# EMI-Group/evogp

Hardware: AMD Instinct MI355X
Metric: tree_evals_per_s (higher is better)
Workload: dtype f32; 1 GPU; BASELINE north_star / configs[2] shape: SymbolicRegression synthetic 10-var, GLOBAL pop=1000000 x 1024 datapoints, max_tree_len=64, funcs + - * /, one tree_SR_fitness pass over every rank's shard per step; global_pop=1000000, pop_per_gpu=1000000, datapoints=1024, var_len=10, max_tree_len=64, ranks=1, device_prewarm_calls=40

## Files before the change

evogp_amd/_lib.py:

```python
from __future__ import annotations

import ctypes as C
import os

_HERE = os.path.dirname(os.path.abspath(__file__))
LIB_PATH = os.environ.get("EVOGP_HIP_LIB") or os.path.join(_HERE, "lib", "libevogp_hip.so")

ABI_VERSION = 9

_vp = C.c_void_p
_u = C.c_uint
_i = C.c_int
_f = C.c_float

PROTOTYPES = {
    "evogp_hip_generate": [_u, _u, _u, _u, _u, _f, _f, _vp, _vp, _vp, _vp, _vp, _vp, _vp, _u, _vp],
    "evogp_hip_mutate": [_i, _i, _vp, _vp, _vp, _vp, _vp, _vp, _vp, _vp, _vp, _vp, _vp],
    "evogp_hip_crossover": [_i, _i, _i, _vp, _vp, _vp, _vp, _vp, _vp, _vp, _vp, _vp, _vp, _vp],
    "evogp_hip_evaluate": [_u, _u, _u, _u, _vp, _vp, _vp, _vp, _vp, _vp],
    "evogp_hip_sr_fitness": [_u, _u, _u, _u, _u, _i, _vp, _vp, _vp, _vp, _vp, _vp, _u, _vp],
    "evogp_hip_generate_masked": [_u, _u, _u, _u, _u, _f, _f, _vp, _vp, _vp, _vp, _vp, _vp, _vp, _u, _vp, _u, _vp],
    "evogp_hip_breed_default": [_i, _i, _i, _i, _vp, _vp, _vp, _vp, _vp, _u, _vp, _vp, _vp, _vp, _vp, _vp, _vp, _vp],
    "evogp_hip_breed_default_rows": [_i, _i, _i, _i, _vp, _vp, _vp, _vp, _vp, _u, _vp, _vp, _vp, _vp, _vp, _vp, _vp, _i, _i, _vp],
    "evogp_hip_breed_default_table": [_i, _i, _i, _i, _i, _vp, _vp, _vp, _vp, _vp, _u, _vp, _vp, _vp, _vp, _vp, _vp, _vp, _i, _i, _vp],
# ... 11 lines not shown
    "evogp_hip_random_words": [C.c_longlong, C.c_longlong, _i, C.c_longlong, C.c_longlong, C.c_longlong, _vp, _vp],
    "evogp_hip_fitness_scores": [_u, _i, _vp, _vp, _vp],
    "evogp_hip_select": [_u, _u, _u, _vp, _vp, _vp, _vp],
    "evogp_hip_select_alternating": [_u, _u, _u, _vp, _vp, _vp, _vp, _vp],
    "evogp_hip_tournament_select": [_u, _u, _u, C.c_longlong, C.c_longlong, _vp, _vp, _vp],
    "evogp_hip_set_program_buffer_limit": [C.c_ulonglong],
    "evogp_hip_release_workspaces": [],
    "evogp_hip_set_allocator": [_vp, _vp],
    "evogp_hip_set_sr_division": [C.c_int],
    "evogp_hip_get_sr_division": [],
    "evogp_hip_abi_version": [],
    "evogp_hip_sr_gradient": [_u, _u, _u, _u, _u, _i, _vp, _vp, _vp, _vp, _vp, _vp, _vp, _vp],
    "evogp_hip_sr_const_step": [_u, _u, _u, _i, _vp, _vp, _vp, _vp, _vp, _vp, _vp, _vp, _vp, _vp],
    "evogp_hip_sr_case_errors": [_u, _u, _u, _u, _u, _i, _vp, _vp, _vp, _vp, _vp, _vp, _vp],
    "evogp_hip_lexicase_workspace_bytes": [_u, _u, _u, C.POINTER(C.c_ulonglong)],
    "evogp_hip_lexicase_select": [_u, _u, _vp, _vp, _u, C.c_longlong, C.c_longlong, _vp, _vp, _vp],
    "evogp_hip_pareto_rank_workspace_bytes": [_u, C.POINTER(C.c_ulonglong)],
    "evogp_hip_pareto_rank": [_u, _u, _vp, _vp, _vp, _vp, _vp, _vp, _vp],
    "evogp_hip_nsga2_select": [_u, _vp, _u, _u, _u, C.c_longlong, C.c_longlong, _vp, _vp],
    "evogp_hip_sr_subtree_errors": [_u, _u, _u, _u, _u, _i, _vp, _vp, _vp, _vp, _vp, _vp, _vp, _vp],
    "evogp_hip_prune_rows": [_u, _u, _u, _i, _i, _vp, _vp, _vp, _vp, _vp, _vp, _vp, _vp, _vp, _vp, _vp],
    "evogp_hip_sr_normal_eq": [_u, _u, _u, _u, _u, _vp, _vp, _vp, _vp, _vp, _vp, _vp, _vp],
    "evogp_hip_sr_lm_step": [_u, _u, _u, _i, _vp, _vp, _vp, _vp, _vp, _vp, _vp, _vp, _vp, _vp],
}

DEBUG_PROTOTYPES = {
    "evogp_hip_timer_begin": [_vp],
    "evogp_hip_timer_end": [_vp, C.POINTER(C.c_float)],
    "evogp_hip_debug_set_stats": [_vp],
    "evogp_hip_debug_compile_batch": [_i],
    "evogp_hip_debug_long_compiler": [_i],
    "evogp_hip_debug_twins": [_i],
    "evogp_hip_debug_tc_fold": [_i],
    "evogp_hip_debug_profile": [_i],
    "evogp_hip_debug_profile_read": [C.POINTER(C.c_float), C.POINTER(C.c_int)],
    "evogp_hip_debug_tc_histogram": [_u, _vp, _i, _vp],
    "evogp_hip_debug_tc_nhandlers": [],
    "evogp_hip_debug_tc_program": [_u, _vp, _i],
    "evogp_hip_debug_forget_function_classes": [],
    "evogp_hip_debug_structural_mutate_given": [_i, _i, _i, _i, _i, _vp, _vp, _vp, _vp, _vp, _vp, _vp, _vp],
    "evogp_hip_debug_insert_mutate_given": [_i, _i, _i, _vp, _vp, _vp, _vp, _vp, _vp, _vp, _vp, _vp, _vp, _vp],
    "evogp_hip_debug_point_mutate_given": [_i, _i, _i, _i, _i, _i, _i, _i, _i, _vp, _vp, _vp, _vp, _vp, _vp, _vp, _vp, _vp, _vp, _vp, _vp, _vp, _vp],
    "evogp_hip_debug_lexicase": [_vp, _i],
    "evogp_hip_debug_pareto_rank": [_i],
}


def _load() -> C.CDLL:
    if not os.path.exists(LIB_PATH):
        raise ImportError(
            f"{LIB_PATH} is missing: build the HIP engine first "
            "(python -c 'import __graft_entry__ as g; g.build()'  or  make -C evogp_amd/csrc). "
            "evogp_amd has no CPU fallback."
        )
    lib = C.CDLL(LIB_PATH)
    for name, argtypes in list(PROTOTYPES.items()) + list(DEBUG_PROTOTYPES.items()):
        fn = getattr(lib, name)
        fn.argtypes = argtypes
        fn.restype = _i
    lib.evogp_hip_evaluate_workspace_bytes.argtypes = [_u, _u]
    lib.evogp_hip_evaluate_workspace_bytes.restype = C.c_size_t
    lib.evogp_hip_select_workspace_bytes.argtypes = []
    lib.evogp_hip_select_workspace_bytes.restype = C.c_size_t
    lib.evogp_hip_program_buffer_bytes.argtypes = []
    lib.evogp_hip_program_buffer_bytes.restype = C.c_ulonglong
    lib.evogp_hip_record_ring_bytes.argtypes = []
# ... 16 lines not shown
```

evogp_amd/csrc/sr_tc.hip:

```cpp
#include "interp.hpp"
#include "launch.hpp"
#include "sr_params.hpp"
#include "tc_interp_k8.inc"
#include "tc_interp_k4.inc"
#include "tc_interp_k1.inc"

#include <atomic>
#include <cstddef>
#include <mutex>
#include <cstdio>
#include <vector>

namespace evogp {

struct TcCompileParams {
    const float *value;
    const int16_t *type;
    const int16_t *size;
    uint2 *prog;
    float *fitness;
    unsigned *marks;
    unsigned *zero_next;
    int pop, gp_len, var_len;
    uint32_t unary_mask;
// ... 2 lines not shown
    uint32_t rec;
    uint32_t overflow;
    int depth;
    int out_len;
    int nblocks;
    int rows;
    int general;
    int heavy_reserve;
    int div_reserve;
    int classify;
    uint32_t recip;
    int twins;
    int long_fast;
    int learn;
    int nan_trees;
};

__device__ inline uint32_t division_in_place(uint32_t id, int after, const TcCompileParams &p) {
    if (id < 24u || id >= 32u) return id;
    const uint32_t form = id - 24u;
    const uint32_t ip = form == 0u ? (uint32_t)EVOGP_TC_H_DIVIP_SS : form == 3u ? (uint32_t)EVOGP_TC_H_DIVIP_SC : form == 4u ? (uint32_t)EVOGP_TC_H_DIVIP_CS : 0u;
    if (ip == 0u) return id;
    const int before = after + (form == 0u ? 1 : 0);
    return before + p.div_reserve <= p.depth ? ip : id;
}

enum : int { TC_S = 0, TC_V = 1, TC_C = 2 };
constexpr int kMarkSampleBlocks = 64;
constexpr int kZeroRounds = 3;
static std::atomic<int> g_long_fast{-1};
static std::atomic<int> g_twins{-1};
static std::atomic<int> g_fold{-1};
static std::atomic<int> g_compile_batch{-2};
static int tc_nan_trees() {
    static const int env_fold = env_int("EVOGP_TC_FOLD", 2);
    const int fo = g_fold.load(std::memory_order_relaxed);
    return fo >= 0 ? fo : (env_fold < 0 || env_fold > 2 ? 2 : env_fold);
}
static_assert(kSentinelHeavy == 0x7FC0FEEDu, "gen/gen_tc_asm.py SENTINEL_HEAVY");

__device__ inline float fold_bin4_fast(int op, float x, float y) {
    return op == 0 ? x + y : op == 1 ? x - y : op == 2 ? x * y : (y == 0.0f ? __builtin_nanf("") : x / y);
}

__device__ inline uint32_t tc_word0(int id, int slot, uint32_t pf_bytes, uint32_t aux = 0u) {
    return ((pf_bytes >> 10) << 24) | ((aux & 0xFFu) << 16) | (uint32_t)(((slot & 1) * EVOGP_TC_NHANDLERS + id) * EVOGP_TC_SLOT);
}

static_assert(EVOGP_TC_H_PUSH_V == EVOGP_TC_H_PUSH_C + 1 && EVOGP_TC_H_DIVIP_CS == EVOGP_TC_H_DIVIP_SS + 2 && EVOGP_TC_H_DIVR_CV == EVOGP_TC_H_DIVR_SV + 2 &&
              EVOGP_TC_H_PUSH_C_NP == EVOGP_TC_H_ADD_SS_NP + 24 && EVOGP_TC_H_DIVIP_SS_NP == EVOGP_TC_H_ADD_SS_NP + 26 &&
              EVOGP_TC_H_DIVR_SV_NP == EVOGP_TC_H_ADD_SS_NP + 29, "gen/gen_tc_asm.py NOPF_TWINS");
__device__ inline int no_prefetch_delta(bool arith3, bool push_c, bool in_place, bool by_recip) {
    return arith3 ? (int)EVOGP_TC_H_ADD_SS_NP : push_c ? (int)EVOGP_TC_H_PUSH_C_NP - (int)EVOGP_TC_H_PUSH_C
         : in_place ? (int)EVOGP_TC_H_DIVIP_SS_NP - (int)EVOGP_TC_H_DIVIP_SS : by_recip ? (int)EVOGP_TC_H_DIVR_SV_NP - (int)EVOGP_TC_H_DIVR_SV : 0;
}
__device__ inline bool next_word_has_variable(const TcCompileParams &, unsigned long long keptwave, bool kept, bool uses_var, bool is_root) {
    const unsigned long long U = __ballot(kept & uses_var);
    return __builtin_amdgcn_inverse_ballot_w64((((~keptwave) + (U << 1)) & keptwave) | __ballot(is_root));
}

__device__ inline void division_by_reciprocal(const TcCompileParams &p, int &id, uint32_t pf, uint32_t d1, uint32_t &aux) {
    const bool sv = id == 3 * 8 + 1, vv = id == 3 * 8 + 5, cv = id == 3 * 8 + 7;
    const bool ok = (p.recip != 0u) & (sv | vv | cv);
    const uint32_t voff = vv ? d1 << 4 : pf;
    aux = ok ? (voff + p.recip) >> 10 : aux;
    id = ok ? (int)EVOGP_TC_H_DIVR_SV + (int)vv + 2 * (int)cv : id;
// ... 378 lines not shown
        Mpz &= B((MU & segmask) == 0ull);
    }
    const M Mhigh = B(hf > p.depth);
    M Mlong = 0ull;
    if (U0) Mlong = Mroot & B(slot + 1 > 31);
    int cls = TREE_OK;
    if ((Min & (~(Mleaf | M4) | Msb | Mhigh | Mlong)) != 0ull) {
        const M segmask = L(Min) ? ((len >= 64 ? ~0ull : ((1ull << len) - 1ull)) << lo) : 0ull;
        auto seg_any = [&](M m) -> bool { return (m & segmask) != 0ull; };
        cls = seg_any(Min & B(kind == 3)) ? TREE_HEAVY : seg_any(Min & B(kind == 5)) ? TREE_GENERAL : seg_any(Min & Msb) ? TREE_HEAVY
            : seg_any(Min & Mhigh) ? (p.gp_len > 64 && p.general ? TREE_GENERAL : TREE_HEAVY) : seg_any(Mlong) ? TREE_HEAVY : TREE_OK;
    }
    const M Mdivown = MB & ~Mpushc & ~Mdivr & B(opx == 3);
    const M Mss = Mdivown & B(form == 0), Msc = Mdivown & B(form == 3), Mcs = Mdivown & B(form == 4);
    const int ip = seli(L(Mss), (int)EVOGP_TC_H_DIVIP_SS, seli(L(Msc), (int)EVOGP_TC_H_DIVIP_SC, (int)EVOGP_TC_H_DIVIP_CS));
    const M Minpl = (Mss | Msc | Mcs) & B(hf + seli(L(Mss), 1, 0) + p.div_reserve <= p.depth);
    id = seli(L(Minpl), ip, id);
    if (p.twins) {
        const M Muses = ~Mpushc & ~MU & ((MB & (MlV | MrV)) | (~MB & MV));
        const M Uk = Mkept & Muses;
        const M nxt = (((~keptwave) + (Uk << 1)) & keptwave) | Mroot;
        id += seli(L(nxt), 0, no_prefetch_delta(L(MB & ~Mpushc & ~Mdivr & B(opx < 3)), L(Mpushc), L(Minpl), L(Mdivr & ~Mpushc)));
    }
    const M Mok = B(cls == TREE_OK);
    if (L(Mkept & Mok & ~Mpz)) *(uint2 *)(rec0 + (roff + (uint32_t)slot * 8u)) = make_uint2(tc_word0(id, slot, pf, aux), d1);
    if (L(Mroot)) {
        uint32_t skip = tc_word0(EVOGP_TC_H_SKIP, 0, 0u), nan_tree = tc_word0(EVOGP_TC_H_NAN_TREE, 0, 0u);
        asm volatile("" : "+v"(skip), "+v"(nan_tree));
        const uint32_t last = selu(L(Mpz), nan_tree, tc_word0(EVOGP_TC_H_END, slot + 1, p.ydelta));
        *(uint2 *)(rec0 + (roff + (uint32_t)seli(L(Mok & ~Mpz), slot + 1, 0) * 8u)) = make_uint2(selu(L(Mok), last, skip), 0u);
    }
    if (cls == TREE_GENERAL && !p.general) cls = TREE_HEAVY;
    return L(Min) ? cls : (int)TREE_OK;
}

template <bool U0>
__device__ inline int compile_pack_arith_plain(const TcCompileParams &p, char *rec0, uint32_t roff, bool in, int lo, int len, int ty, int sz, float val, int lane) {
    auto bperm = [](int v, int i4) -> int { return __builtin_amdgcn_ds_bpermute(i4, v); };
    auto next = [](int v) -> int { return __builtin_amdgcn_update_dpp(0, v, 0x130 , 0xf, 0xf, true); };
    auto any = [](bool c) -> bool { return __builtin_amdgcn_ballot_w64(c) != 0ull; };
    auto seli = [](bool c, int x, int y) -> int { return c ? x : y; };
    auto selu = [](bool c, uint32_t x, uint32_t y) -> uint32_t { return c ? x : y; };
    auto self = [](bool c, float x, float y) -> float { return c ? x : y; };
    const int end = lo + len;
    const uint32_t f = (uint32_t)val;
    const bool isV = ty == T_VAR, isC = ty == T_CONST, isBf = ty == T_BFUNC;
    const uint32_t opu = f - (uint32_t)F_ADD;
    const bool is4 = isBf & (opu < 4u);
    const bool g5 = (isBf & (f - (uint32_t)F_LOOSE_DIV <= (uint32_t)(F_GE - F_LOOSE_DIV))) | (ty == T_TFUNC) | (ty == T_UFUNC);
    const int v = max(0, min((int)val, p.var_len - 1));
    const uint32_t pay = selu(isV, (uint32_t)v * p.var_stride, f2bits(val));
    const bool u0 = U0 && in & (ty == T_UFUNC) & (f - (uint32_t)F_SIN > (uint32_t)(F_LOOSE_SQRT - F_SIN)) & (p.unary_mask != 0u);
    const int kind = seli(isV, 0, seli(isC, 1, seli(is4, 2, seli(u0, 4, seli(g5, 5, 3)))));
    const int op = (int)(opu & 3u);
    const bool isB = in & (kind == 2), isU = U0 && u0;
    const int ks = kind | (sz << 3);
    const int ksl = next(ks);
    const int szl = ksl >> 3;
    const int ri = lane + 1 + szl, ri4 = ri << 2;
    const int ksr = bperm(ks, ri4);
    const int szr = ksr >> 3;
    const bool size_bad = (sz != seli(isB, 1 + szl + szr, seli(isU, 1 + szl, 1))) | (isB & ((szl < 1) | (ri >= end))) | (isU & ((szl < 1) | (lane + 1 >= end)));
    int kl = ksl & 7, kr = ksr & 7;
    uint32_t pl = (uint32_t)next((int)pay), pr = (uint32_t)bperm((int)pay, ri4);
    auto fold = [&](uint32_t a, uint32_t b, bool who) -> uint32_t {
        const float x = bits2f(a), y = bits2f(b);
// ... 1054 lines not shown
                if (ty == T_VAR) {
                    int v = (int)val;
                    v = v < 0 ? 0 : (v >= p.var_len ? p.var_len - 1 : v);
                    pf = (uint32_t)v * p.var_stride; d1 = 0u;
                }
                rec[0] = make_uint2(tc_word0(ty == T_VAR ? EVOGP_TC_H_PUSH_V : EVOGP_TC_H_PUSH_C, 0, pf), d1);
                rec[1] = make_uint2(tc_word0(EVOGP_TC_H_END, 1, p.ydelta), 0u);
            }
            continue;
        }
        if (len <= 0) cls = TREE_BAD;
        else if (len <= 64) {
            if (__any(lane < len && ty == T_UFUNC && p.unary_mask != 0u)) cls = compile_tree<true>(p, rec, len, ty, sz, val, lane);
            else cls = compile_tree_arith(p, rec, len, ty, sz, val, lane);
        }
        if (cls == TREE_GENERAL && !p.general) cls = TREE_HEAVY;
        if (cls != TREE_OK && lane == 0) {
            rec[0] = make_uint2(tc_word0(EVOGP_TC_H_SKIP, 0, 0u), 0u);
            p.fitness[t] = cls == TREE_BAD ? __builtin_nanf("") : bits2f(cls == TREE_GENERAL ? kSentinelGeneral : kSentinelHeavy);
            if (cls == TREE_GENERAL && p.marks) p.marks[4] = 1u;
            else if (cls == TREE_HEAVY && p.marks) {
                p.marks[0] = 1u;
                if (blockIdx.x < kMarkSampleBlocks) atomicAdd(p.marks + 2, 1u);
            }
        }
    }
}

__device__ inline bool generic_node(int ty, float val) {
    const uint32_t f = (uint32_t)val;
    return (ty == T_TFUNC) | ((ty == T_BFUNC) & (f - (uint32_t)F_ADD >= 4u)) | ((ty == T_UFUNC) & ((f == (uint32_t)F_LOOSE_INV) | (f - (uint32_t)F_SINH <= 2u)));
}

template <int B, int MODE, bool LONGROWS>
__global__ __launch_bounds__(256) void tc_compile_packed_kernel(TcCompileParams p) {
    constexpr bool UN = MODE != 0;
    const int lane = threadIdx.x & 63;
    if (p.zero_next && blockIdx.x == 0)
        for (int i = threadIdx.x; i < kCallScratchWords; i += blockDim.x) p.zero_next[i] = 0u;
    const uint32_t wave_id = uni((blockIdx.x * blockDim.x + threadIdx.x) >> 6);
    const uint32_t t0 = wave_id * (uint32_t)B;
    if (t0 >= (uint32_t)p.pop) return;
    const int nb = (int)min((uint32_t)B, (uint32_t)p.pop - t0);
    const int L = p.gp_len;
    int raw = 1;
    if (lane < nb) raw = (int)p.size[(size_t)(t0 + (uint32_t)lane) * L];
    char *const rec0 = (char *)p.prog + (size_t)t0 * p.rec;
    const bool longer = LONGROWS && lane < nb && min(raw, L) > 64;
    if (LONGROWS && longer) {
        uint32_t skip = tc_word0(EVOGP_TC_H_SKIP, 0, 0u);
        asm volatile("" : "+v"(skip));
        *(uint2 *)(rec0 + (uint32_t)__mul24(lane, (int)p.rec)) = make_uint2(skip, 0u);
        p.fitness[t0 + (uint32_t)lane] = bits2f(p.general ? kSentinelGeneral : kSentinelHeavy);
        if (p.marks) {
            if (p.general) {
                const int n = min(raw, L);
                p.marks[p.long_fast ? 8 + (int)(n > 128) + (int)(n > 256) + (int)(n > 512) : 4] = 1u;
            }
            else {
                p.marks[0] = 1u;
                if ((wave_id >> 2) < (uint32_t)kMarkSampleBlocks) atomicAdd(p.marks + 2, 1u);
            }
        }
    }
    const int lens = lane < nb && !longer ? max(1, min(raw, L)) : 0;
    int sval = lens | (raw <= 0 ? 128 : 0) | (lane << 8);
#pragma unroll
    for (int r = 3; r < 7; ++r) {
        const unsigned long long ones = __builtin_amdgcn_ballot_w64((sval & (1 << r)) != 0);
        const int below1 = (int)__builtin_amdgcn_mbcnt_hi((uint32_t)(ones >> 32), __builtin_amdgcn_mbcnt_lo((uint32_t)ones, 0u));
        const int to = (sval & (1 << r)) ? below1 : __popcll(ones) + lane - below1;
        sval = __builtin_amdgcn_ds_permute(to << 2, sval);
    }
    const int slen = sval & 127;
    const size_t node0 = (size_t)t0 * (uint32_t)L;
    const float *const value0 = p.value + node0;
    const int16_t *const type0 = p.type + node0, *const size0 = p.size + node0;
    unsigned long long left = LONGROWS ? __builtin_amdgcn_ballot_w64(slen > 0) : (nb >= 64 ? ~0ull : (1ull << nb) - 1ull);
    bool n_in = false;
    unsigned long long n_inm = 0ull;
    int n_tb = 0, n_lo = 0, n_len = 0, n_bad = 0, n_ty = T_CONST, n_sz = 1;
    float n_val = 0.0f;
    auto plan = [&]() {
        int used = 0, about = 0;
        while (true) {
            const unsigned long long cand = __builtin_amdgcn_ballot_w64(slen <= 64 - used) & left;
            if (cand == 0ull) break;
            const int j = __builtin_ctzll(cand);
            left &= ~(1ull << j);
            const int sv = __builtin_amdgcn_readlane(sval, j), l = sv & 127;
            about = (uint32_t)(lane - used) < (uint32_t)l ? (sv | (used << 16)) : about;
            used += l;
            if (used >= 64) break;
        }
        n_in = lane < used;
        n_inm = used >= 64 ? ~0ull : (1ull << used) - 1ull;
        n_tb = (about >> 8) & 255; n_lo = about >> 16; n_len = about & 127; n_bad = about & 128;
        n_ty = T_CONST; n_sz = 1; n_val = 0.0f;
        if (n_in) {
            const uint32_t at = (uint32_t)(__mul24(n_tb, L) + lane - n_lo);
            n_ty = (int)*(const int16_t *)((const char *)type0 + at * 2u); n_val = *(const float *)((const char *)value0 + at * 4u);
            n_sz = (int)*(const int16_t *)((const char *)size0 + at * 2u);
        }
    };
    bool more = left != 0ull;
    if (more) plan();
    uint32_t seen = 0u;
    while (more) {
        const bool in = n_in;
        const unsigned long long inm = n_inm;
        const int tb = n_tb, lo = n_lo, len = n_len, bad = n_bad, sz = n_sz;
        const int ty = bad ? -1 : n_ty;
        const float val = n_val;
        more = left != 0ull;
        if (more) plan();
        const uint32_t roff = (uint32_t)__mul24(tb, (int)p.rec);
        int cls;
        const bool unary = __builtin_amdgcn_ballot_w64(ty == T_UFUNC) != 0ull;
        if (MODE == 3) cls = compile_pack_mo(p, rec0, roff, in, lo, len, ty, sz, val, lane);
        else if (MODE == 2 && __builtin_amdgcn_ballot_w64(generic_node(ty, val)) != 0ull) cls = compile_pack_generic(p, rec0, roff, in, lo, len, ty, sz, val, lane);
        else if (UN && unary && p.unary_mask != 0u) cls = compile_pack_unary<true>(p, rec0, roff, in, lo, len, ty, sz, val, lane);
        else if (!UN && unary) cls = compile_pack_arith<true>(p, rec0, roff, inm, lo, len, ty, sz, val, lane);
        else cls = compile_pack_arith<false>(p, rec0, roff, inm, lo, len, ty, sz, val, lane);
        if (MODE != 3 && p.learn) {
            const bool look = MODE != 0 || __builtin_amdgcn_ballot_w64(cls != TREE_OK) != 0ull;
            if (look) {
                const bool gen = __builtin_amdgcn_ballot_w64(generic_node(ty, val)) != 0ull;
                const bool un = unary && __builtin_amdgcn_ballot_w64((ty == T_UFUNC) & ((uint32_t)val - (uint32_t)F_SIN <= (uint32_t)(F_LOOSE_SQRT - F_SIN))) != 0ull;
                seen |= ((un | gen) ? 1u : 0u) | (gen ? 2u : 0u);
            }
        }
        if (cls != TREE_OK && in && lane == lo) {
            const bool nan = bad != 0 || cls == TREE_BAD;
            p.fitness[t0 + (uint32_t)tb] = nan ? __builtin_nanf("") : bits2f(cls == TREE_GENERAL ? kSentinelGeneral : kSentinelHeavy);
            if (!nan && p.marks) {
                if (cls == TREE_GENERAL) p.marks[p.long_fast ? 8 : 4] = 1u;
                else {
                    p.marks[0] = 1u;
                    if ((wave_id >> 2) < (uint32_t)kMarkSampleBlocks) atomicAdd(p.marks + 2, 1u);
                }
            }
        }
    }
    if (MODE != 3 && p.learn && p.marks && uni((int)seen) != 0 && lane == 0) {
        p.marks[5] = 1u;
        if (seen & 2u) p.marks[6] = 1u;
    }
}
// ... 980 lines not shown
            long sample = 0;
            for (long w = 0; w < sw && w < n; ++w) sample += (n - 1 - w) / nwaves + 1;
            *mark_sample = (int)sample;
        }
        const size_t clds = 4 * tc_general_lds_bytes(p.gp_len);
        if (clds > 64 * 1024 && !d.attr_set[15]) {
            (void)hipFuncSetAttribute((const void *)tc_compile_general_kernel<true>, hipFuncAttributeMaxDynamicSharedMemorySize, 160 * 1024 - 1024);
            (void)hipGetLastError();
            d.attr_set[15] = true;
        }
        static const int env_packed_env = env_int("EVOGP_TC_PACKED", -1);
        const int set_packed = g_compile_batch.load(std::memory_order_relaxed);
        const int env_packed = set_packed != -2 ? set_packed : env_packed_env;
        static const int env_generic = env_int("EVOGP_TC_PACK_GENERIC", 1);
        const bool packed_mo = p.out_len > 1 && env_packed != 0 && env_generic != 0;
        const bool packed = (p.out_len == 1 && env_packed != 0) || packed_mo;
        if (packed) {
            const bool un = c.nblocks != 1;
            constexpr unsigned kOwnHandlers = (1u << F_ADD) | (1u << F_SUB) | (1u << F_MUL) | (1u << F_DIV) | (1u << F_SIN) | (1u << F_COS) | (1u << F_TAN) |
                                              (1u << F_LOG) | (1u << F_LOOSE_LOG) | (1u << F_EXP) | (1u << F_INV) | (1u << F_NEG) | (1u << F_ABS) |
                                              (1u << F_SQRT) | (1u << F_LOOSE_SQRT);
            const bool may_generic = p.func_mask == 0u || (p.func_mask & ~kOwnHandlers) != 0u;
            const int mode = packed_mo ? 3 : (c.general && p.hint_general && env_generic != 0 && may_generic) ? 2 : (un || c.gp_len > 64) ? 1 : 0;
            int B = n >= 400000 ? 32 : n >= 200000 ? 16 : 8;
            if (env_packed > 0) B = env_packed >= 64 ? 64 : env_packed >= 32 ? 32 : env_packed >= 16 ? 16 : 8;
            if (mode >= 2) B = B >= 16 ? 32 : 8;
            static const int env_pwg = env_int("EVOGP_TC_PACKED_WG", 0);
            const int wgw = env_pwg == 64 ? 1 : env_pwg == 256 ? 4 : n >= 120000 ? 1 : 4;
            const long pblocks = ((long)n + wgw * B - 1) / (wgw * B);
            if (first) *mark_sample = (int)std::min<long>(n, (long)kMarkSampleBlocks * 4 * B);
            learn_packed = c.learn != 0 && mode != 3;
            const dim3 grid((unsigned)pblocks), wg(64 * wgw);
            const bool longrows = c.gp_len > 64;
#define EVOGP_LAUNCH_MODE(BB, MM) \
            do { if (longrows) hipLaunchKernelGGL((tc_compile_packed_kernel<BB, MM, true>), grid, wg, 0, strm, c); \
                 else hipLaunchKernelGGL((tc_compile_packed_kernel<BB, MM, false>), grid, wg, 0, strm, c); } while (0)
#define EVOGP_LAUNCH_PACKED(BB) \
            do { if (mode == 1) EVOGP_LAUNCH_MODE(BB, 1); \
                 else hipLaunchKernelGGL((tc_compile_packed_kernel<BB, 0, false>), grid, wg, 0, strm, c); } while (0)
            if (mode == 3) { if (B == 32) EVOGP_LAUNCH_MODE(32, 3); else EVOGP_LAUNCH_MODE(8, 3); }
            else if (mode == 2) { if (B == 32) EVOGP_LAUNCH_MODE(32, 2); else EVOGP_LAUNCH_MODE(8, 2); }
            else if (B == 64) EVOGP_LAUNCH_PACKED(64);
            else if (B == 32) EVOGP_LAUNCH_PACKED(32);
            else if (B == 16) EVOGP_LAUNCH_PACKED(16);
            else EVOGP_LAUNCH_PACKED(8);
#undef EVOGP_LAUNCH_PACKED
#undef EVOGP_LAUNCH_MODE
        }
        if (packed_mo) {
            hipError_t le = hipGetLastError();
            if (le != hipSuccess) return le;
            if (p.gp_len > 64) launch_marked_general(c, n, strm);
        } else if (p.out_len == 1) {
            if (!packed) hipLaunchKernelGGL(tc_compile_kernel, dim3((unsigned)cblocks), dim3(256), 0, strm, c);
            hipError_t le = hipGetLastError();
            if (le != hipSuccess) return le;
            static const bool dbg_marks = getenv("EVOGP_DEBUG_MARKS") != nullptr;
            if (dbg_marks) {
                std::vector<uint32_t> h((size_t)n);
                (void)hipStreamSynchronize(strm);
                (void)hipMemcpy(h.data(), c.fitness, (size_t)n * 4, hipMemcpyDeviceToHost);
                int shown = 0;
                for (int t = 0; t < n && shown < 4; ++t)
                    if (h[t] == kSentinelGeneral || h[t] == kSentinelHeavy) {
                        std::vector<int16_t> ty(c.gp_len), sz(c.gp_len);
                        std::vector<float> va(c.gp_len);
                        (void)hipMemcpy(ty.data(), c.type + (size_t)t * c.gp_len, c.gp_len * 2, hipMemcpyDeviceToHost);
                        (void)hipMemcpy(sz.data(), c.size + (size_t)t * c.gp_len, c.gp_len * 2, hipMemcpyDeviceToHost);
                        (void)hipMemcpy(va.data(), c.value + (size_t)t * c.gp_len, c.gp_len * 4, hipMemcpyDeviceToHost);
                        fprintf(stderr, "[evogp] tree %d left %s: len %d:", lo + t, h[t] == kSentinelGeneral ? "to the general compiler" : "marked heavy", (int)sz[0]);
                        for (int i = 0; i < sz[0] && i < c.gp_len; ++i) fprintf(stderr, " %d/%g/%d", (int)ty[i], va[i], (int)sz[i]);
// ... 415 lines not shown
#define EVOGP_RUN_TC(F) (wide && k == 8 ? run_tc<8, false, F, true>(p, stream, handled, mark_sample, mark_chunks) \
                        : k == 8 ? run_tc<8, false, F>(p, stream, handled, mark_sample, mark_chunks) \
                        : k == 4 ? run_tc<4, false, F>(p, stream, handled, mark_sample, mark_chunks) \
                                 : run_tc<1, false, F>(p, stream, handled, mark_sample, mark_chunks))
    hipError_t te = dm == 1 ? EVOGP_RUN_TC(1) : dm == 2 ? EVOGP_RUN_TC(2) : EVOGP_RUN_TC(0);
#undef EVOGP_RUN_TC
    if (te == hipSuccess && *handled && env_fused != 0 && fused_ok) fused_keep_spare(stream);
    if (te != hipSuccess || *handled || env_fused == 0 || !fused_ok) return te;
    if (g_prog_limit.load(std::memory_order_relaxed) == 0ull) return te;
    *mark_sample = 0; *mark_chunks = 1;
    return fused();
}

}

extern "C" int evogp_hip_debug_twins(int mode) {
    if (mode < -1 || mode > 1) return EVOGP_E_BADARG;
    evogp::g_twins.store(mode, std::memory_order_relaxed);
    return EVOGP_OK;
}

extern "C" int evogp_hip_debug_tc_fold(int mode) {
    if (mode < -1 || mode > 2) return EVOGP_E_BADARG;
    evogp::g_fold.store(mode, std::memory_order_relaxed);
    return EVOGP_OK;
}

extern "C" int evogp_hip_debug_long_compiler(int fast) {
    if (fast < -1 || fast > 1) return EVOGP_E_BADARG;
    evogp::g_long_fast.store(fast, std::memory_order_relaxed);
    return EVOGP_OK;
}

extern "C" int evogp_hip_debug_compile_batch(int trees) {
    if (trees < -1 || trees > 64) return EVOGP_E_BADARG;
    evogp::g_compile_batch.store(trees, std::memory_order_relaxed);
    return EVOGP_OK;
}

extern "C" int evogp_hip_set_program_buffer_limit(unsigned long long bytes) {
    evogp::g_prog_limit.store(bytes, std::memory_order_relaxed);
    return EVOGP_OK;
}

extern "C" int evogp_hip_set_allocator(evogp_alloc_fn alloc, evogp_free_fn free_fn) {
    if ((alloc == nullptr) != (free_fn == nullptr)) return EVOGP_E_BADARG;
    for (auto &d : evogp::g_tc) {
        std::lock_guard<std::mutex> lock(d.mu);
        if (d.prog || d.graph_prog || !d.retired.empty() || !d.rings.empty() || d.spare_ring) return EVOGP_E_BADARG;
    }
    if (evogp::grad_workspaces_held() || evogp::case_workspaces_held()) return EVOGP_E_BADARG;
    evogp::g_alloc.store(alloc, std::memory_order_release);
    evogp::g_free.store(free_fn, std::memory_order_release);
    return EVOGP_OK;
}

extern "C" unsigned long long evogp_hip_program_buffer_bytes(void) {
    int dev = 0;
    (void)hipGetDevice(&dev);
    evogp::TcDevice &d = evogp::g_tc[dev & 63];
    std::lock_guard<std::mutex> lock(d.mu);
    return (unsigned long long)(d.prog_bytes + d.graph_bytes + d.retired_bytes);
}

extern "C" unsigned long long evogp_hip_record_ring_bytes(void) {
    int dev = 0;
// ... 31 lines not shown
    for (void *r : d.retired) evogp::engine_free(r);
    d.retired.clear(); d.retired_bytes = 0;
    for (auto &r : d.rings) evogp::engine_free(r.buf);
    d.rings.clear();
    if (d.spare_ring) evogp::engine_free(d.spare_ring);
    d.spare_ring = nullptr;
    return (int)e;
}

extern "C" int evogp_hip_debug_tc_histogram(unsigned pop, unsigned long long *device_hist, int hist_len, evogp_stream_t stream) {
    if (!device_hist) return EVOGP_E_NULLPTR;
    return (int)evogp::tc_histogram((int)pop, device_hist, hist_len, (hipStream_t)stream);
}

extern "C" int evogp_hip_debug_tc_nhandlers(void) { return EVOGP_TC_NHANDLERS; }

extern "C" int evogp_hip_debug_tc_program(unsigned tree, unsigned *host_words, int max_words) {
    int dev = 0;
    (void)hipGetDevice(&dev);
    evogp::TcDevice &d = evogp::g_tc[dev & 63];
    std::lock_guard<std::mutex> lock(d.mu);
    if (!d.last_records || (int)tree >= d.last_pop || !host_words) return -1;
    if (hipDeviceSynchronize() != hipSuccess) return -1;
    int n = 0;
    const char *r = d.last_records + (size_t)tree * d.last_rec;
    for (int blk = 0; blk < 64 && n < max_words; ++blk) {
        unsigned w[64];
        if (hipMemcpy(w, r, 256, hipMemcpyDeviceToHost) != hipSuccess) return -1;
        bool more = false;
        for (int i = 0; i < 32 && n < max_words; ++i) {
            const unsigned h = (w[2 * i] & 0xFFFFu) / EVOGP_TC_SLOT, id = h % EVOGP_TC_NHANDLERS;
            if (id == EVOGP_TC_H_NEXT && h < 2u * EVOGP_TC_NHANDLERS) { r += w[2 * i + 1]; more = true; break; }
            host_words[2 * n] = w[2 * i]; host_words[2 * n + 1] = w[2 * i + 1]; ++n;
            if (h >= 2u * EVOGP_TC_NHANDLERS || id == EVOGP_TC_H_END || id == EVOGP_TC_H_END_MO || id == EVOGP_TC_H_END_CLS || id == EVOGP_TC_H_SKIP) break;
        }
        if (!more) break;
    }
    return n;
}
```

include/evogp_hip_debug.h:

```cpp
#ifndef EVOGP_HIP_DEBUG_H
#define EVOGP_HIP_DEBUG_H
#include "evogp_hip.h"
#ifdef __cplusplus
extern "C" {
#endif

int evogp_hip_timer_begin(evogp_stream_t stream);
int evogp_hip_timer_end(evogp_stream_t stream, float *elapsed_ms);

int evogp_hip_debug_set_stats(unsigned long long *device_counters);

int evogp_hip_debug_profile(int enable);
int evogp_hip_debug_profile_read(float *stage_ms , int *calls);

int evogp_hip_debug_compile_batch(int trees);
int evogp_hip_debug_long_compiler(int fast);
int evogp_hip_debug_twins(int mode);
int evogp_hip_debug_tc_fold(int mode);

int evogp_hip_debug_tc_histogram(unsigned pop, unsigned long long *device_hist, int hist_len, evogp_stream_t stream);
int evogp_hip_debug_tc_nhandlers(void);
int evogp_hip_debug_tc_program(unsigned tree, unsigned *host_words, int max_words);

int evogp_hip_debug_forget_function_classes(void);

int evogp_hip_debug_structural_mutate_given(int pop_size, int gp_len, int mode, int inner_is_offset, int skip_rows, const int *given,
                                            const float *value, const int16_t *type, const int16_t *size, float *value_res,
                                            int16_t *type_res, int16_t *size_res, evogp_stream_t stream);
int evogp_hip_debug_insert_mutate_given(int pop_size, int gp_len, int skip_rows, const int *given, const float *value, const int16_t *type,
                                        const int16_t *size, const float *donor_value, const int16_t *donor_type, const int16_t *donor_size,
                                        float *value_res, int16_t *type_res, int16_t *size_res, evogp_stream_t stream);
int evogp_hip_debug_point_mutate_given(int pop_size, int gp_len, int mode, int modify_output, int fix_roulette, int skip_rows, int input_len,
                                       int output_len, int n_consts, const unsigned char *target, const float *u, const int *var_idx,
                                       const int *const_idx, const int *out_idx, const float *value, const int16_t *type, const int16_t *size,
                                       const float *roulette_ufuncs, const float *roulette_bfuncs, const float *roulette_tfuncs,
                                       const float *const_samples, float *value_res, evogp_stream_t stream);

int evogp_hip_debug_lexicase(unsigned long long *device_counters, int stop_after);

int evogp_hip_debug_pareto_rank(int stop_after);

#ifdef __cplusplus
}
#endif
#endif
```

Measured before the change: 1682 billion tree-evals/s.

## Add dense lane-packed compiler path for pure arithmetic trees

Adds a dense compile stage to the packed tree compiler that handles trees made only of + - * / and leaves. Each binary node (or single-leaf tree) is gathered into one wave lane with its two operand payloads, roughly halving the lanes per tree, and a batch is compiled once enough nodes accumulate. Trees that don't fit the pattern fall back to the existing per-node path. It is on by default through the EVOGP_TC_DENSE env var and a debug toggle, and adds extra cross-lane permutes plus a more complex flush schedule.

```diff
diff --git a/evogp_amd/_lib.py b/evogp_amd/_lib.py
--- a/evogp_amd/_lib.py
+++ b/evogp_amd/_lib.py
@@ -67,6 +67,7 @@
     "evogp_hip_debug_long_compiler": [_i],
     "evogp_hip_debug_twins": [_i],
     "evogp_hip_debug_tc_fold": [_i],
+    "evogp_hip_debug_dense_compiler": [_i],
     "evogp_hip_debug_profile": [_i],
     "evogp_hip_debug_profile_read": [C.POINTER(C.c_float), C.POINTER(C.c_int)],
     "evogp_hip_debug_tc_histogram": [_u, _vp, _i, _vp],
diff --git a/evogp_amd/csrc/sr_tc.hip b/evogp_amd/csrc/sr_tc.hip
--- a/evogp_amd/csrc/sr_tc.hip
+++ b/evogp_amd/csrc/sr_tc.hip
@@ -58,6 +58,7 @@
 static std::atomic<int> g_twins{-1};
 static std::atomic<int> g_fold{-1};
 static std::atomic<int> g_compile_batch{-2};
+static std::atomic<int> g_dense{-1};
 static int tc_nan_trees() {
     static const int env_fold = env_int("EVOGP_TC_FOLD", 2);
     const int fo = g_fold.load(std::memory_order_relaxed);
@@ -502,6 +503,190 @@
     }
     if (cls == TREE_GENERAL && !p.general) cls = TREE_HEAVY;
     return L(Min) ? cls : (int)TREE_OK;
+}
+
+__device__ inline bool dense_gather(const TcCompileParams &p, unsigned long long inm, int tb, int lo, int len, int ty, int sz, float val, int lane,
+                                    int &dcnt, uint32_t &dw, uint32_t &dl, uint32_t &dr) {
+    typedef unsigned long long M;
+    auto bperm = [](int v, int i4) -> int { return __builtin_amdgcn_ds_bpermute(i4, v); };
+    auto next = [](int v) -> int { return __builtin_amdgcn_update_dpp(0, v, 0x130 , 0xf, 0xf, true); };
+    auto B = [](bool c) -> M { return __builtin_amdgcn_ballot_w64(c); };
+    auto L = [](M m) -> bool { return __builtin_amdgcn_inverse_ballot_w64(m); };
+    auto seli = [](bool c, int x, int y) -> int { return c ? x : y; };
+    auto selu = [](bool c, uint32_t x, uint32_t y) -> uint32_t { return c ? x : y; };
+    const M Min = inm;
+    const int end = lo + len;
+    const uint32_t f = (uint32_t)val;
+    const M MV = B(ty == T_VAR), MC = B(ty == T_CONST);
+    const uint32_t opu = f - (uint32_t)F_ADD;
+    const M M4 = B(ty == T_BFUNC) & B(opu < 4u);
+    const M MB = Min & M4, Mleaf = MV | MC;
+    const int kind = seli(L(MV), 0, seli(L(MC), 1, 2));
+    const int ks = kind | (sz << 3);
+    const int ksl = next(ks);
+    const int szl = ksl >> 3;
+    const int ri = lane + 1 + szl, ri4 = ri << 2;
+    const int ksr = bperm(ks, ri4);
+    const int szr = ksr >> 3;
+    const M Msb = B(sz != seli(L(MB), 1 + szl + szr, 1)) | (MB & (B(szl < 1) | B(ri >= end)));
+    if ((Min & (~(Mleaf | M4) | Msb)) != 0ull) return false;
+    const int v = max(0, min((int)val, p.var_len - 1));
+    const uint32_t pay = selu(L(MV), (uint32_t)v * p.var_stride, f2bits(val));
+    const uint32_t pl = (uint32_t)next((int)pay), pr = (uint32_t)bperm((int)pay, ri4);
+    const M Mone = Min & B(lane == lo) & Mleaf;
+    const M Mf = MB | Mone;
+    const int rank = (int)__builtin_amdgcn_mbcnt_hi((uint32_t)(Mf >> 32), __builtin_amdgcn_mbcnt_lo((uint32_t)Mf, 0u));
+    const int cnt = __popcll(Mf);
+    const int frank = rank - bperm(rank, lo << 2);
+    const int kl = seli(L(Mone), kind, ksl & 3), kr = seli(L(Mone), 1, ksr & 3);
+    const uint32_t w = (opu & 3u) | ((uint32_t)kl << 2) | ((uint32_t)kr << 4) | selu(L(Mone), 0x80u, 0u) | ((uint32_t)((szl >> 1) & 31) << 8) |
+                       ((uint32_t)tb << 13) | ((uint32_t)(frank & 31) << 19) | ((uint32_t)max(1, len >> 1) << 24);
+    const int to = ((dcnt + seli(L(Mf), rank, cnt + lane - rank)) & 63) << 2;
+    const uint32_t gw = (uint32_t)__builtin_amdgcn_ds_permute(to, (int)w);
+    const uint32_t gl = (uint32_t)__builtin_amdgcn_ds_permute(to, (int)selu(L(Mone), pay, pl));
+    const uint32_t gr = (uint32_t)__builtin_amdgcn_ds_permute(to, (int)pr);
+    const bool mine = (uint32_t)(lane - dcnt) < (uint32_t)cnt;
+    dw = selu(mine, gw, dw); dl = selu(mine, gl, dl); dr = selu(mine, gr, dr);
+    dcnt += cnt;
+    return true;
+}
+
+__device__ inline void compile_dense_arith(const TcCompileParams &p, char *rec0, uint32_t t0, uint32_t wave_id, int cnt, uint32_t w, uint32_t pl, uint32_t pr, int lane) {
+    typedef unsigned long long M;
+    auto bperm = [](int v, int i4) -> int { return __builtin_amdgcn_ds_bpermute(i4, v); };
+    auto next = [](int v) -> int { return __builtin_amdgcn_update_dpp(0, v, 0x130 , 0xf, 0xf, true); };
+    auto B = [](bool c) -> M { return __builtin_amdgcn_ballot_w64(c); };
+    auto L = [](M m) -> bool { return __builtin_amdgcn_inverse_ballot_w64(m); };
+    auto seli = [](bool c, int x, int y) -> int { return c ? x : y; };
+    auto selu = [](bool c, uint32_t x, uint32_t y) -> uint32_t { return c ? x : y; };
+    auto self = [](bool c, float x, float y) -> float { return c ? x : y; };
+    const M Min = cnt >= 64 ? ~0ull : (1ull << cnt) - 1ull;
+    const int op = (int)(w & 3u);
+    int kl = (int)((w >> 2) & 3u), kr = (int)((w >> 4) & 3u);
+    const int tb = (int)((w >> 13) & 63u), frank = (int)((w >> 19) & 31u), dlen = (int)((w >> 24) & 63u);
+    const int lo = lane - frank, end = lo + dlen;
+    const int ri4 = (lane + 1 + (int)((w >> 8) & 31u)) << 2;
+    const uint32_t roff = (uint32_t)__mul24(tb, (int)p.rec);
+    const M Mlf = Min & B((w & 0x80u) != 0u);
+    const M MB = Min & ~Mlf;
+    const M MV = Mlf & B(kl == 0), MC = Mlf & ~MV;
+    const M Mroot = Min & B(frank == 0);
+    const M Mfl = MB & B(kl == 2), Mfr = MB & B(kr == 2);
+    const M Mop0 = B(op == 0), Mop1 = B(op == 1), Mop2 = B(op == 2), Mop3 = B(op == 3);
+    M Mkl1 = B(kl == 1), Mkr1 = B(kr == 1);
+    M MnanL = 0ull, MzL = 0ull, MzR = 0ull;
+    if (p.nan_trees) {
+        const uint32_t ml = pl << 1, mr = pr << 1;
+        MnanL = MB & ((Mkl1 & B(ml > 0xFF000000u)) | (Mkr1 & B(mr > 0xFF000000u)));
+        MzL = MB & Mkl1 & B(ml - 1u >= 0xFF000000u);
+        MzR = MB & Mkr1 & B(mr - 1u >= 0xFF000000u);
+    }
+    auto fold = [&](uint32_t a, uint32_t b, M who) -> uint32_t {
+        const float x = bits2f(a), y = bits2f(b);
+        const float fa = x + y, fs = x - y, fm = x * y;
+        float fd = fm;
+        if ((who & Mop3) != 0ull) fd = self(y == 0.0f, __builtin_nanf(""), x / y);
+        return f2bits(self(L(Mop0), fa, self(L(Mop1), fs, self(L(Mop2), fm, fd))));
+    };
+    const M Mabs = MB & Mkl1 & Mkr1;
+    uint32_t folded = 0u;
+    if (Mabs != 0ull) {
+        folded = selu(L(Mabs), fold(pl, pr, Mabs), 0u);
+        const int ai = seli(L(Mabs), 1, 0);
+        const M Mal = Mfl & B(next(ai) != 0), Mar = Mfr & B(bperm(ai, ri4) != 0);
+        const uint32_t fl = (uint32_t)next((int)folded), fr = (uint32_t)bperm((int)folded, ri4);
+        kl = seli(L(Mal), 1, kl); kr = seli(L(Mar), 1, kr);
+        pl = selu(L(Mal), fl, pl); pr = selu(L(Mar), fr, pr);
+        Mkl1 = B(kl == 1); Mkr1 = B(kr == 1);
+    }
+    const M Mcc = MB & ~Mabs & Mkl1 & Mkr1;
+    uint32_t folded2 = 0u;
+    if (Mcc != 0ull) folded2 = fold(pl, pr, Mcc);
+    const uint32_t cb = pr & 0x7FFFFFFFu, ex = cb >> 23;
+    const M Mdivc = Mop3 & Mkr1;
+    const M Mdz = Mdivc & B(cb == 0u), Mdp = Mdivc & B((cb & 0x007FFFFFu) == 0u) & B(ex - 1u <= 252u);
+    const int opx = seli(L(Mdz | Mdp), 2, op);
+    const uint32_t mirror = (pr & 0x80000000u) | ((254u - ex) << 23);
+    const uint32_t b = selu(L(Mdz), 0x7FC00000u, selu(L(Mdp), mirror, pr));
+    constexpr uint32_t kForms = 5u | (6u << 3) | (2u << 6) | (7u << 9) | (0u << 12) | (4u << 15) | (1u << 18) | (3u << 21) | (0u << 24);
+    const uint32_t pair = min((uint32_t)(kl * 3 + kr), 8u);
+    const int form = (int)((kForms >> (3u * pair)) & 7u);
+    const M MlV = B(kl == 0), MrV = B(kr == 0);
+    const M Mkept = (MB & (~Mabs | Mroot)) | Mlf;
+    const M Mpushc = Mabs | Mcc;
+    const int leaf_id = seli(L(MV), (int)EVOGP_TC_H_PUSH_V, (int)EVOGP_TC_H_PUSH_C);
+    const M Mdivr = MB & Mop3 & MrV & (p.recip != 0u ? ~0ull : 0ull);
+    const uint32_t aux = selu(L(Mdivr), (pr + p.recip) >> 10, 0u);
+    const int fn_id = seli(L(Mdivr), (int)EVOGP_TC_H_DIVR_SV + ((form * 3) >> 3), opx * 8 + form);
+    int id = seli(L(Mpushc), (int)EVOGP_TC_H_PUSH_C, seli(L(MB), fn_id, leaf_id));
+    const uint32_t pf = selu(L(Mpushc), 0u, selu(L(MB), selu(L(MlV), pl, selu(L(MrV), pr, 0u)), selu(L(MV), pl, 0u)));
+    const uint32_t d1B = selu(L(Mkl1), pl, selu(L(Mkr1), b, selu(L(MlV & MrV), b >> 4, 0u)));
+    const uint32_t d1 = selu(L(Mabs), folded, selu(L(Mcc), folded2, selu(L(MB), d1B, selu(L(MV), 0u, pl))));
+    const int kepti = seli(L(Mkept), 1, 0);
+    const int deltaB = (int)(kl != 2) + (int)(kr != 2) - 1;
+    const int deltaf = seli(L(Mabs), kepti, seli(L(MB), deltaB, seli(L(Mlf), 1, 0)));
+    const M keptwave = Mkept;
+    const int above = __popcll(keptwave) - (int)__builtin_amdgcn_mbcnt_hi((uint32_t)(keptwave >> 32), __builtin_amdgcn_mbcnt_lo((uint32_t)keptwave, 0u)) - kepti;
+    const int inclf = wave_scan_incl(deltaf);
+    M Mnan = 0ull;
+    if (p.nan_trees) {
+        const M Mconst = MC | Mabs | Mcc;
+        const uint32_t mag2 = d1 << 1;
+        Mnan = (Mconst & B(mag2 > 0xFF000000u)) | (MB & Mdz) | MnanL;
+        if (p.nan_trees >= 2) {
+            const M Z0 = (Mconst & B(mag2 - 1u >= 0xFF000000u)) | (MB & Mop1 & MlV & MrV & B(pl == pr));
+            const int zleft = seli(L(MB & (Mop2 | Mop3)), 1, 0);
+            const int zboth = seli(L(MB & (Mop0 | Mop1)), 1, 0);
+            const int zright = seli(L(MB & Mop2), 1, 0);
+            const int zL = seli(L(MzL), 1, 0), zR = seli(L(MzR), 1, 0), mL = seli(L(Mfl), 1, 0), mR = seli(L(Mfr), 1, 0);
+            int z = seli(L(Z0), 1, 0);
+            int zr = zR | (bperm(z, ri4) & mR);
+#pragma unroll
+            for (int r = 0; r < kZeroRounds; ++r) {
+                const int zl = zL | (next(z) & mL);
+                z |= (zl & ((zr & zboth) | zleft)) | (zr & zright);
+                zr = zR | (bperm(z, ri4) & mR);
+            }
+            Mnan |= MB & Mop3 & B(zr != 0);
+        }
+    }
+    const int nanincl = (int)__builtin_amdgcn_mbcnt_hi((uint32_t)(Mnan >> 32), __builtin_amdgcn_mbcnt_lo((uint32_t)Mnan, 0u)) + seli(L(Mnan), 1, 0);
+    const int both = (int)((uint32_t)inclf << 15) | (nanincl << 8) | above;
+    const int at_end = bperm(both, (end - 1) << 2), before = bperm(both, (lo - 1) << 2);
+    const int base = seli(lo > 0, before >> 15, 0);
+    const int slot = above - (at_end & 0xFF);
+    const int totf = (at_end >> 15) - base;
+    const int hf = seli(L(Mkept), totf - (inclf - base - deltaf), 0);
+    const M Mpz = Min & B(((at_end >> 8) & 127) != seli(lo > 0, (before >> 8) & 127, 0));
+    const M Mhigh = Min & B(hf > p.depth);
+    M Mdeep = 0ull;
+    if (Mhigh != 0ull) Mdeep = Min & B((Mhigh & (((1ull << dlen) - 1ull) << (lo & 63))) != 0ull);
+    const M Mdivown = MB & ~Mpushc & ~Mdivr & B(opx == 3);
+    const M Mss = Mdivown & B(form == 0), Msc = Mdivown & B(form == 3), Mcs = Mdivown & B(form == 4);
+    const int ip = seli(L(Mss), (int)EVOGP_TC_H_DIVIP_SS, seli(L(Msc), (int)EVOGP_TC_H_DIVIP_SC, (int)EVOGP_TC_H_DIVIP_CS));
+    const M Minpl = (Mss | Msc | Mcs) & B(hf + seli(L(Mss), 1, 0) + p.div_reserve <= p.depth);
+    id = seli(L(Minpl), ip, id);
+    if (p.twins) {
+        const M Muses = ~Mpushc & ((MB & (MlV | MrV)) | MV);
+        const M Uk = Mkept & Muses;
+        const M nxt = (((~keptwave) + (Uk << 1)) & keptwave) | Mroot;
+        id += seli(L(nxt), 0, no_prefetch_delta(L(MB & ~Mpushc & ~Mdivr & B(opx < 3)), L(Mpushc), L(Minpl), L(Mdivr & ~Mpushc)));
+    }
+    const M Mok = ~Mdeep;
+    if (L(Mkept & Mok & ~Mpz)) *(uint2 *)(rec0 + (roff + (uint32_t)slot * 8u)) = make_uint2(tc_word0(id, slot, pf, aux), d1);
+    if (L(Mroot)) {
+        uint32_t skip = tc_word0(EVOGP_TC_H_SKIP, 0, 0u), nan_tree = tc_word0(EVOGP_TC_H_NAN_TREE, 0, 0u);
+        asm volatile("" : "+v"(skip), "+v"(nan_tree));
+        const uint32_t last = selu(L(Mpz), nan_tree, tc_word0(EVOGP_TC_H_END, slot + 1, p.ydelta));
+        *(uint2 *)(rec0 + (roff + (uint32_t)seli(L(Mok & ~Mpz), slot + 1, 0) * 8u)) = make_uint2(selu(L(Mok), last, skip), 0u);
+    }
+    if (L(Mroot & Mdeep)) {
+        p.fitness[t0 + (uint32_t)tb] = bits2f(kSentinelHeavy);
+        if (p.marks) {
+            p.marks[0] = 1u;
+            if ((wave_id >> 2) < (uint32_t)kMarkSampleBlocks) atomicAdd(p.marks + 2, 1u);
+        }
+    }
 }
 
 template <bool U0>
@@ -1622,8 +1807,9 @@
     return (ty == T_TFUNC) | ((ty == T_BFUNC) & (f - (uint32_t)F_ADD >= 4u)) | ((ty == T_UFUNC) & ((f == (uint32_t)F_LOOSE_INV) | (f - (uint32_t)F_SINH <= 2u)));
 }
 
-template <int B, int MODE, bool LONGROWS>
+template <int B, int MODE, bool LONGROWS, bool DENSE = false>
 __global__ __launch_bounds__(256) void tc_compile_packed_kernel(TcCompileParams p) {
+    static_assert(!DENSE || (MODE == 0 && !LONGROWS), "the dense word stage is the arithmetic line's");
     constexpr bool UN = MODE != 0;
     const int lane = threadIdx.x & 63;
     if (p.zero_next && blockIdx.x == 0)
@@ -1670,19 +1856,22 @@
     bool n_in = false;
     unsigned long long n_inm = 0ull;
     int n_tb = 0, n_lo = 0, n_len = 0, n_bad = 0, n_ty = T_CONST, n_sz = 1;
+    int n_need = 0;
     float n_val = 0.0f;
     auto plan = [&]() {
-        int used = 0, about = 0;
+        int used = 0, about = 0, need = 0;
         while (true) {
-            const unsigned long long cand = __builtin_amdgcn_ballot_w64(slen <= 64 - used) & left;
+            const unsigned long long cand = __builtin_amdgcn_ballot_w64(DENSE ? (slen <= 64 - used) & (((slen + 1) >> 1) <= 32 - need) : slen <= 64 - used) & left;
             if (cand == 0ull) break;
             const int j = __builtin_ctzll(cand);
             left &= ~(1ull << j);
             const int sv = __builtin_amdgcn_readlane(sval, j), l = sv & 127;
             about = (uint32_t)(lane - used) < (uint32_t)l ? (sv | (used << 16)) : about;
             used += l;
+            need += (l + 1) >> 1;
             if (used >= 64) break;
         }
+        n_need = need;
         n_in = lane < used;
         n_inm = used >= 64 ? ~0ull : (1ull << used) - 1ull;
         n_tb = (about >> 8) & 255; n_lo = about >> 16; n_len = about & 127; n_bad = about & 128;
@@ -1696,6 +1885,12 @@
     bool more = left != 0ull;
     if (more) plan();
     uint32_t seen = 0u;
+    int dcnt = 0;
+    uint32_t dw = 0u, dl = 0u, dr = 0u;
+    auto dense_flush = [&]() {
+        compile_dense_arith(p, rec0, t0, wave_id, dcnt, dw, dl, dr, lane);
+        dcnt = 0;
+    };
     while (more) {
         const bool in = n_in;
         const unsigned long long inm = n_inm;
@@ -1704,6 +1899,11 @@
         const float val = n_val;
         more = left != 0ull;
         if (more) plan();
+        if (DENSE) {
+            const bool taken = dense_gather(p, inm, tb, lo, len, ty, sz, val, lane, dcnt, dw, dl, dr);
+            if (dcnt > 0 && (!more || dcnt + n_need > 64)) dense_flush();
+            if (taken) continue;
+        }
         const uint32_t roff = (uint32_t)__mul24(tb, (int)p.rec);
         int cls;
         const bool unary = __builtin_amdgcn_ballot_w64(ty == T_UFUNC) != 0ull;
@@ -2750,11 +2950,15 @@
             learn_packed = c.learn != 0 && mode != 3;
             const dim3 grid((unsigned)pblocks), wg(64 * wgw);
             const bool longrows = c.gp_len > 64;
+            static const int env_dense = env_int("EVOGP_TC_DENSE", 1);
+            const int set_dense = g_dense.load(std::memory_order_relaxed);
+            const bool dense = (set_dense >= 0 ? set_dense : env_dense) != 0;
 #define EVOGP_LAUNCH_MODE(BB, MM) \
             do { if (longrows) hipLaunchKernelGGL((tc_compile_packed_kernel<BB, MM, true>), grid, wg, 0, strm, c); \
                  else hipLaunchKernelGGL((tc_compile_packed_kernel<BB, MM, false>), grid, wg, 0, strm, c); } while (0)
 #define EVOGP_LAUNCH_PACKED(BB) \
             do { if (mode == 1) EVOGP_LAUNCH_MODE(BB, 1); \
+                 else if (dense) hipLaunchKernelGGL((tc_compile_packed_kernel<BB, 0, false, true>), grid, wg, 0, strm, c); \
                  else hipLaunchKernelGGL((tc_compile_packed_kernel<BB, 0, false>), grid, wg, 0, strm, c); } while (0)
             if (mode == 3) { if (B == 32) EVOGP_LAUNCH_MODE(32, 3); else EVOGP_LAUNCH_MODE(8, 3); }
             else if (mode == 2) { if (B == 32) EVOGP_LAUNCH_MODE(32, 2); else EVOGP_LAUNCH_MODE(8, 2); }
@@ -3236,6 +3440,12 @@
     return EVOGP_OK;
 }
 
+extern "C" int evogp_hip_debug_dense_compiler(int mode) {
+    if (mode < -1 || mode > 1) return EVOGP_E_BADARG;
+    evogp::g_dense.store(mode, std::memory_order_relaxed);
+    return EVOGP_OK;
+}
+
 extern "C" int evogp_hip_debug_compile_batch(int trees) {
     if (trees < -1 || trees > 64) return EVOGP_E_BADARG;
     evogp::g_compile_batch.store(trees, std::memory_order_relaxed);
@@ -3333,7 +3543,7 @@
             const unsigned h = (w[2 * i] & 0xFFFFu) / EVOGP_TC_SLOT, id = h % EVOGP_TC_NHANDLERS;
             if (id == EVOGP_TC_H_NEXT && h < 2u * EVOGP_TC_NHANDLERS) { r += w[2 * i + 1]; more = true; break; }
             host_words[2 * n] = w[2 * i]; host_words[2 * n + 1] = w[2 * i + 1]; ++n;
-            if (h >= 2u * EVOGP_TC_NHANDLERS || id == EVOGP_TC_H_END || id == EVOGP_TC_H_END_MO || id == EVOGP_TC_H_END_CLS || id == EVOGP_TC_H_SKIP) break;
+            if (h >= 2u * EVOGP_TC_NHANDLERS || id == EVOGP_TC_H_END || id == EVOGP_TC_H_END_MO || id == EVOGP_TC_H_END_CLS || id == EVOGP_TC_H_SKIP || id == EVOGP_TC_H_NAN_TREE) break;
         }
         if (!more) break;
     }
diff --git a/include/evogp_hip_debug.h b/include/evogp_hip_debug.h
--- a/include/evogp_hip_debug.h
+++ b/include/evogp_hip_debug.h
@@ -17,6 +17,7 @@
 int evogp_hip_debug_long_compiler(int fast);
 int evogp_hip_debug_twins(int mode);
 int evogp_hip_debug_tc_fold(int mode);
+int evogp_hip_debug_dense_compiler(int mode);
 
 int evogp_hip_debug_tc_histogram(unsigned pop, unsigned long long *device_hist, int hist_len, evogp_stream_t stream);
 int evogp_hip_debug_tc_nhandlers(void);
```

Measured after the change: 1741 billion tree-evals/s (median of 6 runs). 3.5% higher.
